# stecrotti/MPSKit.jl

Measured on AMD Instinct MI355X. Metric: DMRG sweeps/sec + ddAC matvec achieved-TFLOP/s, Heisenberg L=100 D=1024 fp64, higher is better.
Workload: dtype f64; 1 GPU; Heisenberg S=1/2 FiniteMPS L=100 D=1024 d=2 W=5 fp64, 1-site DMRG sweep (2L-2 site updates), fixed Krylov budget 8 matvecs/site; parallelism=single GPU

## Files before the change

mpskit.jl_amd/csrc/mpsk_cholqr.hip:

```cpp
#include <hip/hip_runtime.h>
#include <cmath>
#include <cstdio>
#include <cstdlib>
#include <cstring>
#include <string>
#include "mpsk_internal.h"

namespace mpsk {

constexpr int CB = 64;
constexpr double CQ_FIRSTORDER_MAX = 1.0e-7;

__global__ __launch_bounds__(256) void cq_pad_identity_kernel(double* __restrict__ G, int npad, int n) {
  const int64_t total = (int64_t)npad * npad;
  for (int64_t e = blockIdx.x * (int64_t)blockDim.x + threadIdx.x; e < total; e += (int64_t)gridDim.x * blockDim.x) {
    int r = (int)(e % npad), c = (int)(e / npad);
    if (r >= n || c >= n) G[e] = (r == c) ? 1.0 : 0.0;
  }
}

__global__ __launch_bounds__(256) void cq_shift_kernel(double* __restrict__ G, int npad, int n, double factor) {
  __shared__ double red[4];
  __shared__ double sh;
  double acc = 0.0;
// ... 461 lines not shown
    double v = G[r + (int64_t)c * npad] - (r == c ? 1.0 : 0.0);
    if (!(fabs(v) <= thresh)) bad = 1;
  }
  if (bad) atomicOr(flag, 2);
}

static bool cq_use_trsm(int m, int npad) {
  static const bool enabled = !(getenv("MPSK_CQ_TRSM") && atoi(getenv("MPSK_CQ_TRSM")) == 0);
  return enabled && (int64_t)(npad / CB) * ((m + CB - 1) / CB) <= 768;
}
static bool cq_use_gram(int m, int npad) {
  static const bool enabled = !(getenv("MPSK_CQ_GRAM") && atoi(getenv("MPSK_CQ_GRAM")) == 0);
  return enabled && cq_use_trsm(m, npad);
}

size_t cholqr_workspace_doubles(int m, int n) {
  int nb = (n + CB - 1) / CB, p2 = 1;
  while (p2 < nb) p2 <<= 1;
  size_t npad = (size_t)p2 * CB;
  return 5 * npad * npad + 2 * (size_t)m * n + 16 + (cq_use_gram(m, (int)npad) ? (size_t)CQ_GS * npad * npad : 0);
}

static GemmArgs cq_mk(const double* A, const double* B, double* C, int M, int N, int K, int64_t lda, int64_t ldb,
                      int64_t ldc, int tA, double alpha, double beta) {
  GemmArgs g;
  std::memset(&g, 0, sizeof(g));
  g.A = A; g.B = B; g.C = C; g.M = M; g.N = N; g.K = K; g.lda = lda; g.ldb = ldb; g.ldc = ldc;
  g.batch = 1; g.nseg = 1; g.alpha = alpha; g.beta = beta; g.transA = tA; g.transB = 0;
  return g;
}

static hipError_t cq_pass(int m, int n, int npad, const double* X, int ldx, double* Q, int ldq, double* Rp,
                          double* Rinv, double* T, bool shifted, bool check_identity, int* flag, hipStream_t s,
                          double shift_scale = 1.0, bool gram_ready = false, double* Gp_next = nullptr) {
  hipError_t e;
  double* Gw = T;
  GemmArgs g = cq_mk(X, X, Gw, n, n, m, ldx, ldx, npad, 1, 1.0, 0.0);
  g.upper_only = 1;
  if (!gram_ready && (e = gemm_f64(g, s)) != hipSuccess) return e;
  if (npad > n) hipLaunchKernelGGL(cq_pad_identity_kernel, dim3(512), dim3(256), 0, s, Gw, npad, n);
  if (check_identity) hipLaunchKernelGGL(cq_check_identity_kernel, dim3(256), dim3(256), 0, s, Gw, npad, n, 0.5, flag);
  if (shifted) {
    const double u = 1.1102230246251565e-16;
    const double factor = shift_scale * 11.0 * ((double)m * n + (double)n * (n + 1)) * u;
    hipLaunchKernelGGL(cq_shift_kernel, dim3(1), dim3(256), 0, s, Gw, npad, n, factor);
  }
  const int nb = npad / CB;
  static std::atomic<uint64_t> step_attr{0};
  if ((e = ensure_dyn_smem(step_attr, reinterpret_cast<const void*>(cq_step_kernel), CQ_STEP_LDS)) != hipSuccess) return e;
  const bool use_trsm = cq_use_trsm(m, npad);
  if (use_trsm) {
    if (X != Q) {
      if ((e = hipMemcpy2DAsync(Q, sizeof(double) * (size_t)ldq, X, sizeof(double) * (size_t)ldx, sizeof(double) * (size_t)m, n,
                                hipMemcpyDeviceToDevice, s)) != hipSuccess) return e;
    }
    const int mt = (m + CB - 1) / CB;
    for (int k = 0; k <= nb + (Gp_next ? 2 : 1); ++k) {
      const int nt = (nb - k > 0) ? nb - k : 0;
      int nwg = (k == 0) ? 1 : nt * (nt + 1) / 2 + nt;
      if (k - 2 >= 0 && k - 2 < nb) nwg += mt;
      if (k - 3 >= 0 && nb - k + 1 > 0) nwg += (nb - k + 1) * mt;
      if (Gp_next && k - 3 >= 0 && k - 3 < nb) nwg += (k - 2) * CQ_GS;
      if (nwg > 0)
        hipLaunchKernelGGL(cq_step_kernel, dim3(nwg), dim3(256), CQ_STEP_LDS, s, Gw, Rp, Rinv, npad, k, flag, Q, m, n, ldq, 1,
                           Gp_next);
    }
    hipLaunchKernelGGL(cq_cleanup_kernel, dim3(1024), dim3(256), 0, s, Rp, Rinv, npad);
    if (Gp_next) hipLaunchKernelGGL(cq_gram_reduce_kernel, dim3(1024), dim3(256), 0, s, Gp_next, npad, T);
    return hipGetLastError();
  }
  for (int k = 0; k <= nb; ++k) {
    const int nt = nb - k;
    const int pairwg = (k >= 2 && (k & 1) == 0) ? 1 : 0;
    const int nwg = (k == 0) ? 1 : nt * (nt + 1) / 2 + nt + pairwg;
    if (nwg > 0)
      hipLaunchKernelGGL(cq_step_kernel, dim3(nwg), dim3(256), CQ_STEP_LDS, s, Gw, Rp, Rinv, npad, k, flag, (double*)nullptr, 0, 0, 0, 0,
                         (double*)nullptr);
  }
  hipLaunchKernelGGL(cq_cleanup_kernel, dim3(1024), dim3(256), 0, s, Rp, Rinv, npad);
  for (int b = 2 * CB; b < npad; b <<= 1) {
    const int pairs = npad / (2 * b);
    const int64_t bs = (int64_t)2 * b * (npad + 1);
    const int64_t off12 = (int64_t)b * npad;
    const int64_t off22 = (int64_t)b * (npad + 1);
    g = cq_mk(Rp + off12, Rinv + off22, T + off12, b, b, b, npad, npad, npad, 0, 1.0, 0.0);
    g.batch = pairs; g.bsA = bs; g.bsB = bs; g.bsC = bs;
    if ((e = gemm_f64(g, s)) != hipSuccess) return e;
    g = cq_mk(Rinv, T + off12, Rinv + off12, b, b, b, npad, npad, npad, 0, -1.0, 0.0);
    g.batch = pairs; g.bsA = bs; g.bsB = bs; g.bsC = bs;
    if ((e = gemm_f64(g, s)) != hipSuccess) return e;
  }
  g = cq_mk(X, Rinv, Q, m, n, n, ldx, npad, ldq, 0, 1.0, 0.0);
  g.b_upper = 1;
  return gemm_f64(g, s);
}

__global__ __launch_bounds__(256) void cq_copy_upper_kernel(const double* __restrict__ Rp, int npad, int n,
                                                            double* __restrict__ R, int ldr) {
  const int64_t total = (int64_t)n * n;
// ... 16 lines not shown
      if (!(fabs(ev) <= 1.0e-7)) big = 1;
      u = (r < c) ? ev : 0.5 * ev;
    }
    R3[e] = id + u;
    Minv[e] = id - u;
  }
  if (big) atomicOr(flag, 4);
}

static hipError_t cq_pass_firstorder(int m, int n, int npad, const double* X, int ldx, double* Q, int ldq, double* Rp,
                                     double* Rinv, double* T, int* flag, hipStream_t s, bool gram_ready = false) {
  hipError_t e;
  GemmArgs g = cq_mk(X, X, T, n, n, m, ldx, ldx, npad, 1, 1.0, 0.0);
  g.upper_only = 1;
  if (!gram_ready && (e = gemm_f64(g, s)) != hipSuccess) return e;
  hipLaunchKernelGGL(cq_firstorder_kernel, dim3(1024), dim3(256), 0, s, T, npad, n, Rp, Rinv, flag, CQ_FIRSTORDER_MAX);
  g = cq_mk(X, Rinv, Q, m, n, n, ldx, npad, ldq, 0, 1.0, 0.0);
  g.b_upper = 1;
  return gemm_f64(g, s);
}

struct CqBufs { double *R1, *R2, *R3, *Rinv, *T, *Qa, *Qb, *Gp; int npad; };
static CqBufs cq_bufs(int m, int n, double* ws) {
  int nb = (n + CB - 1) / CB, p2 = 1;
  while (p2 < nb) p2 <<= 1;
  CqBufs b;
  b.npad = p2 * CB;
  const size_t np2 = (size_t)b.npad * b.npad;
  b.R1 = ws; b.R2 = b.R1 + np2; b.R3 = b.R2 + np2; b.Rinv = b.R3 + np2; b.T = b.Rinv + np2;
  b.Qa = b.T + np2; b.Qb = b.Qa + (size_t)m * n;
  b.Gp = cq_use_gram(m, b.npad) ? b.Qb + (((size_t)m * n + 1) & ~(size_t)1) : nullptr;
  return b;
}
static hipError_t cq_finish(const CqBufs& b, int n, double* R, int ldr, int* d_flag, int* flag_out, hipStream_t s) {
  hipError_t e;
  GemmArgs g = cq_mk(b.R2, b.R1, b.T, b.npad, b.npad, b.npad, b.npad, b.npad, b.npad, 0, 1.0, 0.0);
  g.a_upper = g.b_upper = g.upper_only = 1;
  if ((e = gemm_f64(g, s)) != hipSuccess) return e;
  g = cq_mk(b.R3, b.T, b.Rinv, b.npad, b.npad, b.npad, b.npad, b.npad, b.npad, 0, 1.0, 0.0);
  g.a_upper = g.b_upper = g.upper_only = 1;
  if ((e = gemm_f64(g, s)) != hipSuccess) return e;
  hipLaunchKernelGGL(cq_copy_upper_kernel, dim3(1024), dim3(256), 0, s, b.Rinv, b.npad, n, R, ldr);
  return hipMemcpyAsync(flag_out, d_flag, sizeof(int), hipMemcpyDeviceToHost, s);
}

static void cq_dbg_count(bool rep) {
  static long n = 0, r = 0;
  if (!getenv("MPSK_CQ_DEBUG")) return;
  ++n; if (rep) ++r;
  if (n % 100 == 0) fprintf(stderr, "[cholqr3] %ld factorizations, %ld repeated the third pass (thr %.1e)\n", n, r, CQ_FIRSTORDER_MAX);
}
hipError_t cholqr3_enqueue(int m, int n, const double* A, int lda, double* Q, int ldq, double* R, int ldr, double* ws,
                           int* d_flag, int* flag_out, hipStream_t s, double shift_scale) {
  const CqBufs b = cq_bufs(m, n, ws);
  hipError_t e;
  if ((e = hipMemsetAsync(d_flag, 0, sizeof(int), s)) != hipSuccess) return e;
  const bool gr = (b.Gp != nullptr);
  if ((e = cq_pass(m, n, b.npad, A, lda, b.Qa, m, b.R1, b.Rinv, b.T, true, false, d_flag, s, shift_scale, false, b.Gp)) != hipSuccess) return e;
  if ((e = cq_pass(m, n, b.npad, b.Qa, m, b.Qb, m, b.R2, b.Rinv, b.T, false, false, d_flag, s, 1.0, gr, b.Gp)) != hipSuccess) return e;
  if ((e = cq_pass_firstorder(m, n, b.npad, b.Qb, m, Q, ldq, b.R3, b.Rinv, b.T, d_flag, s, gr)) != hipSuccess) return e;
  return cq_finish(b, n, R, ldr, d_flag, flag_out, s);
}

hipError_t cholqr3_finalize(int m, int n, double* Q, int ldq, double* R, int ldr, double* ws, int* d_flag,
                            int* flag_out, hipStream_t s) {
  const CqBufs b = cq_bufs(m, n, ws);
  hipError_t e;
  if ((e = hipStreamSynchronize(s)) != hipSuccess) return e;
  cq_dbg_count(*flag_out == 4);
  if (*flag_out == 4) {
    if ((e = hipMemsetAsync(d_flag, 0, sizeof(int), s)) != hipSuccess) return e;
    if ((e = cq_pass(m, n, b.npad, b.Qb, m, Q, ldq, b.R3, b.Rinv, b.T, false, true, d_flag, s)) != hipSuccess) return e;
    if ((e = cq_finish(b, n, R, ldr, d_flag, flag_out, s)) != hipSuccess) return e;
    if ((e = hipStreamSynchronize(s)) != hipSuccess) return e;
  }
  return hipGetLastError();
}

__global__ __launch_bounds__(256) void cq_sumsq_kernel(const double* __restrict__ A, int lda, int m, int n,
                                                       double* __restrict__ out) {
  __shared__ double red[4];
  const int64_t total = (int64_t)m * n;
  double acc = 0.0;
  for (int64_t e = blockIdx.x * (int64_t)blockDim.x + threadIdx.x; e < total; e += (int64_t)gridDim.x * blockDim.x) {
    const double v = A[(e % m) + (e / m) * (int64_t)lda];
    acc += v * v;
  }
  for (int off = 32; off > 0; off >>= 1) acc += __shfl_down(acc, off, 64);
  if ((threadIdx.x & 63) == 0) red[threadIdx.x >> 6] = acc;
  __syncthreads();
  if (threadIdx.x == 0) out[1 + blockIdx.x] = red[0] + red[1] + red[2] + red[3];
}
__global__ __launch_bounds__(64) void cq_sumsq_final_kernel(double* __restrict__ out, int nblocks) {
  if (threadIdx.x == 0) {
    double acc = 0.0;
    for (int i = 0; i < nblocks; ++i) acc += out[1 + i];
    out[0] = acc;
  }
}
__global__ __launch_bounds__(256) void cq_perturb_kernel(const double* __restrict__ A, int lda, int m, int n,
                                                         double* __restrict__ X, int ldx, const double* __restrict__ sumsq) {
  const double delta = 1.1102230246251565e-16 * sqrt(sumsq[0] / (double)m);
  const int64_t total = (int64_t)m * n;
  for (int64_t e = blockIdx.x * (int64_t)blockDim.x + threadIdx.x; e < total; e += (int64_t)gridDim.x * blockDim.x) {
// ... 72 lines not shown
```

mpskit.jl_amd/csrc/mpsk_gemm.hip:

```cpp
#include <hip/hip_runtime.h>
#include <stdint.h>
#include <cstdio>
#include <cstdlib>
#include <cstring>
#include <map>
#include <mutex>
#include <string>
#include <vector>
#include "mpsk_internal.h"

namespace mpsk {

typedef double d4 __attribute__((ext_vector_type(4)));
typedef double d2 __attribute__((ext_vector_type(2)));

constexpr int BK = 16;
constexpr int NTHREADS = 256;

template <int BMN, bool KMAJOR> struct LdsImg {
  static_assert(BK == 16, "the K-major swizzle assumes 128-byte rows");
  static constexpr int STRIDE = KMAJOR ? BK : (BMN + 16);
  static constexpr int SIZE = KMAJOR ? BMN * BK : BK * (BMN + 16);
  __device__ static inline int idx(int mn, int k) { return KMAJOR ? mn * BK + (k ^ (mn & 15)) : k * STRIDE + mn; }
};
// ... 320 lines not shown
    const int rm = tilesM / g.xcd_gx, rn = tilesN / g.xcd_gy;
    const int xi = xcd % g.xcd_gx, yi = xcd / g.xcd_gx;
    const int ln = pos / rm, lm = pos - ln * rm;
    *bm = xi * rm + lm;
    *bn = yi * rn + ln;
    (void)rn;
  } else {
    *bn = t / tilesM;
    *bm = t - *bn * tilesM;
  }
}

template <int BM, int BN, bool ALIGNED, bool CJ = false, bool ZADD = false>
__device__ __forceinline__ void gemm_store_c(const GemmArgs& g, double* __restrict__ Cb, int z, int m0, int n0,
                                             const d4 (&acc)[BM / 32][BN / 32]) {
  constexpr int WTM = BM / 2, WTN = BN / 2, TM = WTM / 16, TN = WTN / 16;
  const int lane = threadIdx.x & 63, wave = threadIdx.x >> 6;
  const int wm = wave & 1, wn = wave >> 1, fr = lane & 15, fq = lane >> 4;
  const double alpha = g.alpha, beta = g.beta;
#pragma unroll
  for (int i = 0; i < TM; ++i) {
    const int m = m0 + wm * WTM + i * 16 + fr;
#pragma unroll
    for (int j = 0; j < TN; ++j) {
#pragma unroll
      for (int rg = 0; rg < 4; ++rg) {
        const int n = n0 + wn * WTN + j * 16 + fq + 4 * rg;
        if (ALIGNED || (m < g.M && n < g.N)) {
          const int64_t mo = CJ ? (int64_t)m * g.c_rs : (int64_t)m;
          double* p = (g.tabC2 != nullptr && n >= g.splitN)
                          ? g.C + g.tabC2[z] + mo + (int64_t)(n - g.splitN) * g.ldc
                          : Cb + mo + (int64_t)n * g.ldc;
          double v = alpha * acc[i][j][rg];
          if constexpr (ZADD) v += g.gamma * g.Z[(int64_t)m + (int64_t)n * g.ldz];
          else if (beta != 0.0) v += beta * (*p);
          *p = v;
        }
      }
    }
  }
}

template <int BM, int BN>
__device__ __forceinline__ void gemm_store_ws(double alpha, double* __restrict__ slot, const d4 (&acc)[BM / 32][BN / 32]) {
  constexpr int WTM = BM / 2, WTN = BN / 2, TM = WTM / 16, TN = WTN / 16;
  const int lane = threadIdx.x & 63, wave = threadIdx.x >> 6;
  const int wm = wave & 1, wn = wave >> 1, fr = lane & 15, fq = lane >> 4;
#pragma unroll
  for (int i = 0; i < TM; ++i)
#pragma unroll
    for (int j = 0; j < TN; ++j)
#pragma unroll
      for (int rg = 0; rg < 4; ++rg)
        slot[(wm * WTM + i * 16 + fr) + (wn * WTN + j * 16 + fq + 4 * rg) * BM] = alpha * acc[i][j][rg];
}

template <int BM, int BN, bool TA, bool TB, bool ALIGNED, bool ZS = false, bool CJ = false, bool ZADD = false>
__device__ __forceinline__ void gemm_body(const GemmArgs& g) {
  extern __shared__ __attribute__((aligned(16))) double smem[];
  const int tilesM = (g.M + BM - 1) / BM, tilesN = (g.N + BN - 1) / BN;
  const int ntiles = tilesM * tilesN;
  int bid = blockIdx.x;
  if (!g.xcd_interleave) {
    int q = ntiles / 8, r = ntiles % 8, xcd = bid % 8, pos = bid / 8;
    bid = (xcd < r ? xcd * (q + 1) : r * (q + 1) + (xcd - r) * q) + pos;
  }
  int bm, bn;
  tile_coords(g, bid, tilesM, tilesN, &bm, &bn);
  const int z = blockIdx.y;
  if (g.upper_only && bm > bn && (g.upper_nb == 0 || z < g.upper_nb)) return;
  const int m0 = bm * BM, n0 = bn * BN;
  const double* Ab = g.A + (g.tabA ? g.tabA[z] : (int64_t)z * g.bsA);
  const double* Bb = g.B + (g.tabB ? g.tabB[z] : (int64_t)z * g.bsB);
  double* Cb = g.C + (g.tabC ? g.tabC[z] : (int64_t)z * g.bsC);
  d4 acc[BM / 32][BN / 32];
#pragma unroll
  for (int i = 0; i < BM / 32; ++i)
#pragma unroll
    for (int j = 0; j < BN / 32; ++j) acc[i][j] = d4{0.0, 0.0, 0.0, 0.0};
  const int nt = ((g.K + BK - 1) / BK) * g.nseg;
  int ktlo = 0, kthi = nt;
  if (g.b_upper) { const int lim = (n0 + BN + BK - 1) / BK; if (lim < kthi) kthi = lim; }
  if (g.a_upper) ktlo = m0 / BK;
  if (ktlo < kthi) gemm_acc_dispatch<BM, BN, TA, TB, ALIGNED, ZS, CJ>(g, Ab, Bb, z, m0, n0, ktlo, kthi, acc, smem);
  gemm_store_c<BM, BN, ALIGNED, CJ, ZADD>(g, Cb, z, m0, n0, acc);
}

template <int BM, int BN, bool TA, bool TB, bool ALIGNED, bool ZS = false, bool ZADD = false>
__device__ __forceinline__ void gemm_sk_body(const GemmArgs& g) {
  extern __shared__ __attribute__((aligned(16))) double smem[];
  constexpr int WTM = BM / 2, WTN = BN / 2, TM = WTM / 16, TN = WTN / 16;
  const int tilesM = (g.M + BM - 1) / BM, tilesN = (g.N + BN - 1) / BN;
  const int ntiles = tilesM * tilesN;
  const int KT = ((g.K + BK - 1) / BK) * g.nseg;
  const int U = ntiles * g.batch * KT;
  int sid = blockIdx.x;
  if (!g.xcd_interleave) {
    const int nwg = gridDim.x;
    int q = nwg / 8, r = nwg % 8, xcd = sid % 8, pos = sid / 8;
    sid = (xcd < r ? xcd * (q + 1) : r * (q + 1) + (xcd - r) * q) + pos;
  }
  int u = sid * g.sk_units;
  int slot = sid;
  if (g.sk_split_major) {
    const int TZ = ntiles * g.batch;
    const int split = sid / TZ, tzs = sid - split * TZ;
    u = tzs * KT + split * g.sk_units;
    slot = tzs * (KT / g.sk_units - 1) + split - 1;
  }
  const int uend = (u + g.sk_units < U) ? u + g.sk_units : U;
  const int lane = threadIdx.x & 63, wave = threadIdx.x >> 6;
  const int wm = wave & 1, wn = wave >> 1, fr = lane & 15, fq = lane >> 4;
  while (u < uend) {
    const int tz = u / KT;
    const int kt0 = u - tz * KT;
    const int kt1 = (uend - u < KT - kt0) ? kt0 + (uend - u) : KT;
    const int z = tz / ntiles, tile = tz - z * ntiles;
    int bm, bn;
// ... 97 lines not shown
      for (int q = 0; q < UNR; ++q) {
        const int e = e0 + 256 * q;
        if (e < eend) sacc[q] += g.sk_ws[(int64_t)(g.sk_split_major ? w - tz - 1 : w) * BM * BN + e];
      }
    }
#pragma unroll
    for (int q = 0; q < UNR; ++q)
      if (pp[q]) *pp[q] = cv[q] + sacc[q];
  }
}

template <int BM, int BN, bool TA, bool TB, bool ALIGNED>
__global__ __launch_bounds__(NTHREADS, min_waves(BM, BN)) void gemm_f64_kernel(GemmArgs g) {
  gemm_body<BM, BN, TA, TB, ALIGNED>(g);
}

template <int BM, int BN, bool ALIGNED>
__global__ __launch_bounds__(NTHREADS, min_waves(BM, BN)) void dac_gemm_f64_kernel(GemmArgs g) {
  gemm_body<BM, BN, false, false, ALIGNED>(g);
}
template <int BM, int BN, bool ALIGNED>
__global__ __launch_bounds__(NTHREADS, min_waves(BM, BN)) void dac_gemm_zs_f64_kernel(GemmArgs g) {
  gemm_body<BM, BN, false, false, ALIGNED, true>(g);
}

template <int BM, int BN, bool ALIGNED>
__global__ __launch_bounds__(NTHREADS, min_waves(BM, BN)) void gemm_tn_zadd_f64_kernel(GemmArgs g) {
  gemm_body<BM, BN, true, false, ALIGNED, false, false, true>(g);
}
template <int BM, int BN, bool ALIGNED>
__global__ __launch_bounds__(NTHREADS, min_waves(BM, BN)) void gemm_tn_zadd_sk_f64_kernel(GemmArgs g) {
  gemm_sk_body<BM, BN, true, false, ALIGNED, false, true>(g);
}

template <int BM, int BN, bool TA, bool TB, bool ALIGNED>
__global__ __launch_bounds__(NTHREADS, min_waves(BM, BN)) void cgemm_f64_kernel(GemmArgs g) {
  gemm_body<BM, BN, TA, TB, ALIGNED, false, true>(g);
}

struct ProfRec { hipEvent_t e0, e1; double flops; int bm, bn, aligned, sk, zs; };
static std::atomic<bool> g_prof_on{false};
static std::atomic<uint64_t> g_prof_seq{0};
static const int g_prof_stride = getenv("MPSK_PROF_STRIDE") && atoi(getenv("MPSK_PROF_STRIDE")) > 0 ? atoi(getenv("MPSK_PROF_STRIDE")) : 1;
static std::mutex g_prof_mu;
static std::vector<ProfRec> g_prof;

void gemm_prof_enable(bool on) {
  std::lock_guard<std::mutex> lk(g_prof_mu);
  if (on && !g_prof_on.load()) {
    for (auto& r : g_prof) { (void)hipEventDestroy(r.e0); (void)hipEventDestroy(r.e1); }
    g_prof.clear();
  }
  if (on) g_prof_seq.store(0);
  g_prof_on.store(on);
}
static void prof_push(const ProfRec& r) {
  std::lock_guard<std::mutex> lk(g_prof_mu);
  g_prof.push_back(r);
}

std::string gemm_prof_summary() {
  (void)hipDeviceSynchronize();
  struct Agg { long n = 0; double ms = 0, flops = 0; };
  std::map<std::string, Agg> agg;
  std::lock_guard<std::mutex> lk(g_prof_mu);
  for (auto& r : g_prof) {
// ... 26 lines not shown
  if (hipError_t e = ensure_dyn_smem(attr, reinterpret_cast<const void*>(kern), smem); e != hipSuccess) return e;
  if (prof) {
    (void)hipEventCreateWithFlags(&r->e0, hipEventDisableSystemFence); (void)hipEventCreateWithFlags(&r->e1, hipEventDisableSystemFence);
    (void)hipEventRecord(r->e0, s);
  }
  hipLaunchKernelGGL(kern, grid, dim3(NTHREADS), smem, s, g);
  return hipGetLastError();
}

template <int BM, int BN, bool TA, bool TB, bool ALIGNED>
static hipError_t launch_cfg(const GemmArgs& g, hipStream_t s) {
  using LA = TileLoader<BM, TA, ALIGNED>;
  using LB = TileLoader<BN, !TB, ALIGNED>;
  constexpr size_t smem = (2 * LA::Img::SIZE + 2 * LB::Img::SIZE) * sizeof(double);
  const int tilesM = (g.M + BM - 1) / BM, tilesN = (g.N + BN - 1) / BN;
  dim3 grid(tilesM * tilesN, g.batch, 1);
  const bool zs = g.zsegA != nullptr;
  if (zs && !(g.tag == 1 && !TA && !TB && g.zsegB != nullptr)) return hipErrorInvalidValue;
  const bool tagged = (g.tag == 1 && !TA && !TB);
  bool prof = tagged && g_prof_on.load(std::memory_order_relaxed);
  if (prof) {
    const uint64_t n = g_prof_seq.fetch_add(1, std::memory_order_relaxed);
    prof = ((n >> 1) % (uint64_t)g_prof_stride) == 0;
  }
  ProfRec r;
  r.flops = 2.0 * g.M * g.N * (double)g.K * g.nseg * g.batch; r.bm = BM; r.bn = BN; r.aligned = ALIGNED; r.sk = 0; r.zs = zs;
  hipError_t e = hipSuccess;
  if (g.cplx) {
    if (zs || g.sk_units > 0) return hipErrorInvalidValue;
    static std::atomic<uint64_t> c0{0};
    return launch_one(cgemm_f64_kernel<BM, BN, TA, TB, ALIGNED>, c0, grid, smem, g, s, false, &r);
  }
  constexpr bool ZADD_OK = TA && !TB;
  if (g.Z && !ZADD_OK) return hipErrorInvalidValue;
  if constexpr ((BM == 128 && BN == 128) || (BM == 64 && BN == 64)) {
    if (g.sk_units > 0) {
      const int KT = ((g.K + BK - 1) / BK) * g.nseg;
      const int64_t U = (int64_t)tilesM * tilesN * g.batch * KT;
      const dim3 sgrid((unsigned)((U + g.sk_units - 1) / g.sk_units));
      r.sk = 1;
      static std::atomic<uint64_t> a0{0}, a1{0}, a2{0}, a3{0};
      if constexpr (ZADD_OK) {
        if (g.Z) e = launch_one(gemm_tn_zadd_sk_f64_kernel<BM, BN, ALIGNED>, a3, sgrid, smem, g, s, false, &r);
        else e = launch_one(gemm_sk_f64_kernel<BM, BN, TA, TB, ALIGNED>, a0, sgrid, smem, g, s, false, &r);
      } else if constexpr (!TA && !TB) {
        if (tagged && zs) e = launch_one(dac_gemm_sk_zs_f64_kernel<BM, BN, ALIGNED>, a2, sgrid, smem, g, s, prof, &r);
        else if (tagged) e = launch_one(dac_gemm_sk_f64_kernel<BM, BN, ALIGNED>, a1, sgrid, smem, g, s, prof, &r);
        else e = launch_one(gemm_sk_f64_kernel<BM, BN, TA, TB, ALIGNED>, a0, sgrid, smem, g, s, false, &r);
      } else {
        e = launch_one(gemm_sk_f64_kernel<BM, BN, TA, TB, ALIGNED>, a0, sgrid, smem, g, s, false, &r);
      }
      if (e != hipSuccess) return e;
      hipLaunchKernelGGL((gemm_sk_fixup_kernel<BM, BN>), dim3(tilesM * tilesN * g.batch, (BM * BN) / 1024), dim3(256), 0, s, g);
      if (prof) { (void)hipEventRecord(r.e1, s); prof_push(r); }
      return hipGetLastError();
    }
  }
  static std::atomic<uint64_t> b0{0}, b1{0}, b2{0}, b3{0};
  if constexpr (ZADD_OK) {
    if (g.Z) e = launch_one(gemm_tn_zadd_f64_kernel<BM, BN, ALIGNED>, b3, grid, smem, g, s, false, &r);
    else e = launch_one(gemm_f64_kernel<BM, BN, TA, TB, ALIGNED>, b0, grid, smem, g, s, false, &r);
  } else if constexpr (!TA && !TB) {
    if (tagged && zs) e = launch_one(dac_gemm_zs_f64_kernel<BM, BN, ALIGNED>, b2, grid, smem, g, s, prof, &r);
    else if (tagged) e = launch_one(dac_gemm_f64_kernel<BM, BN, ALIGNED>, b1, grid, smem, g, s, prof, &r);
    else e = launch_one(gemm_f64_kernel<BM, BN, TA, TB, ALIGNED>, b0, grid, smem, g, s, false, &r);
  } else {
    e = launch_one(gemm_f64_kernel<BM, BN, TA, TB, ALIGNED>, b0, grid, smem, g, s, false, &r);
// ... 37 lines not shown
  std::lock_guard<std::mutex> lk(g_skws_mu);
  SkWs& e = g_skws[std::make_pair(dev, s)];
  if (e.p) return e.p;
  if (hipMalloc(&e.p, SK_WS_DOUBLES * sizeof(double)) != hipSuccess) { e.p = nullptr; return nullptr; }
  return e.p;
}
void gemm_retain_stream(hipStream_t s) {
  int dev = 0;
  if (hipGetDevice(&dev) != hipSuccess) return;
  std::lock_guard<std::mutex> lk(g_skws_mu);
  g_skws[std::make_pair(dev, s)].refs++;
}
void gemm_release_stream(hipStream_t s) {
  int dev = 0;
  if (hipGetDevice(&dev) != hipSuccess) return;
  double* p = nullptr;
  {
    std::lock_guard<std::mutex> lk(g_skws_mu);
    auto it = g_skws.find(std::make_pair(dev, s));
    if (it == g_skws.end()) return;
    if (--it->second.refs > 0) return;
    p = it->second.p;
    g_skws.erase(it);
  }
  if (p) { (void)hipStreamSynchronize(s); (void)hipFree(p); }
}

hipError_t gemm_f64(const GemmArgs& g_in, hipStream_t s) {
  GemmArgs g = g_in;
  if (g.M <= 0 || g.N <= 0 || g.batch <= 0) return hipSuccess;
  if (g.K <= 0 || g.nseg <= 0) {
    return hipErrorInvalidValue;
  }
  if (g.Z && (!g.transA || g.transB || g.cplx || g.tabC2 || g.batch != 1 || g.beta != 0.0 || g.Z == g.C || g.zsegA))
    return hipErrorInvalidValue;
  if (!g.A2 && !g.B2) { g.A2 = g.A; g.B2 = g.B; g.nseg1 = g.nseg; }
  else if (!g.A2 || !g.B2 || !g.zsegA || !g.zsegB || g.nseg1 < 0 || g.nseg1 > g.nseg) return hipErrorInvalidValue;
  int bm = 128, bn = 128;
  choose_tile(g.M, g.N, g.K * g.nseg, g.batch, &bm, &bn);
  g.sk_units = 0;
  g.sk_ws = nullptr;
  g.sk_split_major = 0;
  if (g.cplx && g.c_rs == 0) g.c_rs = 1;
  if (g.upper_only && g.M != g.N) g.upper_only = 0;
  if (g.nseg != 1 || g.transA || g.transB) g.a_upper = g.b_upper = 0;
  if (g_force_bm.load()) { bm = g_force_bm.load(); bn = g_force_bn.load(); }
  else if (g.cplx) {  }
  else {
    const int KT = ((g.K + BK - 1) / BK) * g.nseg;
    const int64_t Tb = (int64_t)((g.M + 127) / 128) * ((g.N + 127) / 128) * g.batch;
    const int64_t Ts = (int64_t)((g.M + 63) / 64) * ((g.N + 63) / 64) * g.batch;
    if (g_sk_enabled) {
      const int64_t Ub = Tb * KT;
      if (Tb >= 128 && Tb < 4 * 512 && Tb % 512 != 0 && Ub / 512 >= 16) {
        double* ws = sk_workspace(s);
        if (ws) { bm = bn = 128; g.sk_units = (int)((Ub + 511) / 512); g.sk_ws = ws; }
      }
    }
    if (g.sk_units == 0 && g_splitk_enabled && bm == 64 && bn == 64 && KT >= 64 && Ts <= 4096) {
      const int64_t slots = (int64_t)(SK_WS_DOUBLES / (64 * 64));
      int best_f = 1;
      double best = 0.0;
      for (int f = 1; f <= 8; ++f) {
        if (f > 1 && (KT / f < 16 || Ts * (f - 1) > slots)) break;
        const int64_t n = (Ts * f + 255) / 256;
        const int r = (int)(n % 4);
        const double phi[4] = {1.0, 0.55, 0.92, 0.98};
        const double len = (double)KT / f + 6.0;
        const double cost = (double)(n - r) * len + (r ? r * len / phi[r] : 0.0) + 3.0 * (f - 1) * (double)n / f + (f > 1 ? 12.0 : 0.0);
        if (f == 1 || cost < 0.97 * best) { best = cost; best_f = f; }
      }
      if (g_splitk_force > 0 && (g_splitk_force == 1 || (KT / g_splitk_force >= 16 && Ts * (g_splitk_force - 1) <= slots)))
        best_f = g_splitk_force;
      if (best_f >= 2) {
        double* ws = sk_workspace(s);
        if (ws) {
          g.sk_units = (KT + best_f - 1) / best_f;
          g.sk_ws = ws;
          g.sk_split_major = (KT % g.sk_units == 0 && KT / g.sk_units == best_f) ? 1 : 0;
          if (!g.sk_split_major) {
// ... 7 lines not shown
  g.xcd_interleave = (g.upper_only || g.a_upper || g.b_upper) ? 1 : 0;
  {
    const int tM = (g.M + bm - 1) / bm, tN = (g.N + bn - 1) / bn;
    g.xcd_gx = g.xcd_gy = 0;
    const bool chunks_ok = ((int64_t)tM * tN) % 8 == 0 &&
                           (g.sk_units == 0 || (((g.K + BK - 1) / BK) * g.nseg) % g.sk_units == 0);
    if (chunks_ok && g_xcd_grid_enabled && !g.xcd_interleave) {
      double best = 0.0;
      const int cand[4][2] = {{1, 8}, {2, 4}, {4, 2}, {8, 1}};
      for (int c = 0; c < 4; ++c) {
        if (tM % cand[c][0] || tN % cand[c][1]) continue;
        const double cost = (double)g.M / cand[c][0] + (double)g.N / cand[c][1];
        if (g.xcd_gx == 0 || cost < best) { best = cost; g.xcd_gx = cand[c][0]; g.xcd_gy = cand[c][1]; }
      }
    }
  }
  bool aligned = (g.M % bm == 0) && (g.N % bn == 0) && (g.K % BK == 0) && (g.lda % 2 == 0) &&
                 (g.ldb % 2 == 0) && (g.bsA % 2 == 0) && (g.bsB % 2 == 0) &&
                 ((uintptr_t)g.A % 16 == 0) && ((uintptr_t)g.B % 16 == 0) &&
                 ((uintptr_t)g.A2 % 16 == 0) && ((uintptr_t)g.B2 % 16 == 0) &&
                 g.lda < ((int64_t)1 << 21) && g.ldb < ((int64_t)1 << 21);
  if (g.tabA || g.tabB || g.zsegA || g.zsegB) aligned = aligned && g.tabs_even;
  if (!g.zsegA) for (int i = 0; i < g.nseg && i < MAXSEG; ++i) aligned = aligned && (g.segA[i] % 2 == 0);
  if (!g.zsegB) for (int i = 0; i < g.nseg && i < MAXSEG; ++i) aligned = aligned && (g.segB[i] % 2 == 0);
  if ((!g.zsegA || !g.zsegB) && g.nseg > MAXSEG) return hipErrorInvalidValue;
  if (g.upper_only && bm != bn) g.upper_only = 0;
#define MPSK_DISPATCH(TA_, TB_)                                                        \
  return aligned ? launch_tile<TA_, TB_, true>(g, bm, bn, s) : launch_tile<TA_, TB_, false>(g, bm, bn, s)
  if (!g.transA && !g.transB) { MPSK_DISPATCH(false, false); }
  if (g.transA && !g.transB) { MPSK_DISPATCH(true, false); }
  if (!g.transA && g.transB) { MPSK_DISPATCH(false, true); }
  MPSK_DISPATCH(true, true);
#undef MPSK_DISPATCH
}

template <int BM, bool ALIGNED, bool TWO> struct PairLoader {
  using L = TileLoader<BM, false, ALIGNED>;
  using Img = typename L::Img;
  static constexpr int NV = L::NV;
  L p, q;
  double c[NV][4];

  __device__ inline void load(const GemmPairArgs& g, int m0, int k0, int tid) {
    p.load(g.P, g.ldp, m0, k0, g.M, g.K, tid);
    if (g.Q) q.load(g.Q, g.ldq, m0, k0, g.M, g.K, tid);
#pragma unroll
    for (int i = 0; i < NV; ++i) {
      const int gk = k0 + (tid + i * NTHREADS) / (BM / 2);
      const bool in = ALIGNED || gk < g.K;
      if (!g.Q) q.r[i] = d2{0.0, 0.0};
      c[i][0] = in ? g.a1[gk] : 0.0;
      c[i][1] = (in && g.Q) ? g.b1[gk] : 0.0;
      c[i][2] = (TWO && in) ? g.a2[gk] : 0.0;
      c[i][3] = (TWO && in && g.Q) ? g.b2[gk] : 0.0;
    }
  }
  __device__ inline void store(double* __restrict__ lds, int tid) const {
#pragma unroll
    for (int i = 0; i < NV; ++i) {
      const int v = tid + i * NTHREADS;
      const int mn = (v % (BM / 2)) * 2, k = v / (BM / 2);
      const d2 pv = p.r[i], qv = q.r[i];
      *reinterpret_cast<d2*>(&lds[Img::idx(mn, k)]) = d2{pv.x * c[i][0] + qv.x * c[i][1], pv.y * c[i][0] + qv.y * c[i][1]};
      if (TWO)
        *reinterpret_cast<d2*>(&lds[Img::SIZE + Img::idx(mn, k)]) =
            d2{pv.x * c[i][2] + qv.x * c[i][3], pv.y * c[i][2] + qv.y * c[i][3]};
// ... 381 lines not shown
```

mpskit.jl_amd/csrc/mpsk_internal.h:

```cpp
#pragma once
#include <hip/hip_runtime.h>
#include <stdint.h>
#include <stddef.h>
#include <atomic>
#include <vector>
#include <string>

namespace mpsk {

inline hipError_t ensure_dyn_smem(std::atomic<uint64_t>& done, const void* kernel, size_t bytes) {
  int dev = 0;
  hipError_t e = hipGetDevice(&dev);
  if (e != hipSuccess) return e;
  const uint64_t bit = 1ull << (dev & 63);
  if (done.load(std::memory_order_acquire) & bit) return hipSuccess;
  e = hipFuncSetAttribute(kernel, hipFuncAttributeMaxDynamicSharedMemorySize, (int)bytes);
  if (e != hipSuccess) return e;
  done.fetch_or(bit, std::memory_order_release);
  return hipSuccess;
}

constexpr int MAXSEG = 32;

struct GemmArgs {
// ... 4 lines not shown
  int64_t lda, ldb, ldc;
  int64_t bsA, bsB, bsC;
  int batch;
  int nseg;
  int64_t segA[MAXSEG], segB[MAXSEG];
  double alpha, beta;
  int transA, transB;
  const int64_t* tabA;
  const int64_t* tabB;
  const int64_t* tabC;
  const int64_t* tabC2;
  int splitN;
  int sk_units;
  int sk_split_major;
  double* sk_ws;
  int xcd_gx, xcd_gy;
  int xcd_interleave;
  const int64_t* zsegA;
  const int64_t* zsegB;
  const double* A2;
  const double* B2;
  int nseg1;
  signed char segJ[MAXSEG];
  int b_upper, a_upper;
  int upper_only;
  int upper_nb;
  int cplx;
  int c_rs;
  int tag;
  int tabs_even;
  const double* Z;
  int64_t ldz;
  double gamma;
};

hipError_t gemm_f64(const GemmArgs& g, hipStream_t s);
void gemm_force_tile(int bm, int bn);
void gemm_retain_stream(hipStream_t s);
void gemm_release_stream(hipStream_t s);
void gemm_enable_streamk(bool on);
void gemm_prof_enable(bool on);
std::string gemm_prof_summary();

struct GemmPairArgs {
  const double* P;
  const double* Q;
  const double* B;
  double* C1;
  double* C2;
  int M, N, K;
  int64_t ldp, ldq, ldb, ld1, ld2;
  const double* a1;
  const double* b1;
  const double* a2;
  const double* b2;
  double beta1, beta2;
};
hipError_t gemm_pair_f64(const GemmPairArgs& g, hipStream_t s);
struct DsumArgs {
  GemmArgs f[2];
  int rmod[2];
  int64_t rstride;
  int ntiles0;
};
static_assert(sizeof(DsumArgs) <= 4096, "DsumArgs is passed by value as a kernel argument");
hipError_t dsum_f64(const DsumArgs& a, hipStream_t s);
hipError_t grassmann_coef(int K, const double* S, double scalar, int mode, double* coef, hipStream_t s);

struct MixTerm { int32_t out, in; double coef; double coef_im = 0.0; };
// ... 96 lines not shown
```

Before: 1.165 sweeps/s.

## Fuse CholeskyQR3 tail: first-order pass, grouped GEMMs, triangular R output

Adds a fused tail path for CholeskyQR3 when the Gram-accumulation buffer exists. The second pass skips its cleanup and Gram-reduce launches, and one kernel reduces the partial Gram, builds the first-order R3 and its inverse, and sets the repeat flag. The Q GEMM and the R2*R1 GEMM then run together in one grouped launch, and the final R3*T product writes straight into R with the lower triangle zeroed (new c_tri epilogue in an NN zadd GEMM path). This removes several kernel launches and a copy kernel per factorization. In exchange it adds new GEMM variants, and the fallback path now needs an extra cleanup launch.

```diff
diff --git a/mpskit.jl_amd/csrc/mpsk_cholqr.hip b/mpskit.jl_amd/csrc/mpsk_cholqr.hip
--- a/mpskit.jl_amd/csrc/mpsk_cholqr.hip
+++ b/mpskit.jl_amd/csrc/mpsk_cholqr.hip
@@ -517,7 +517,8 @@
 
 static hipError_t cq_pass(int m, int n, int npad, const double* X, int ldx, double* Q, int ldq, double* Rp,
                           double* Rinv, double* T, bool shifted, bool check_identity, int* flag, hipStream_t s,
-                          double shift_scale = 1.0, bool gram_ready = false, double* Gp_next = nullptr) {
+                          double shift_scale = 1.0, bool gram_ready = false, double* Gp_next = nullptr,
+                          bool fused_tail = false) {
   hipError_t e;
   double* Gw = T;
   GemmArgs g = cq_mk(X, X, Gw, n, n, m, ldx, ldx, npad, 1, 1.0, 0.0);
@@ -550,6 +551,7 @@
         hipLaunchKernelGGL(cq_step_kernel, dim3(nwg), dim3(256), CQ_STEP_LDS, s, Gw, Rp, Rinv, npad, k, flag, Q, m, n, ldq, 1,
                            Gp_next);
     }
+    if (fused_tail && Gp_next) return hipGetLastError();
     hipLaunchKernelGGL(cq_cleanup_kernel, dim3(1024), dim3(256), 0, s, Rp, Rinv, npad);
     if (Gp_next) hipLaunchKernelGGL(cq_gram_reduce_kernel, dim3(1024), dim3(256), 0, s, Gp_next, npad, T);
     return hipGetLastError();
@@ -632,6 +634,48 @@
   b.Gp = cq_use_gram(m, b.npad) ? b.Qb + (((size_t)m * n + 1) & ~(size_t)1) : nullptr;
   return b;
 }
+static bool cq_use_tail() {
+  static const bool enabled = !(getenv("MPSK_CQ_TAIL") && atoi(getenv("MPSK_CQ_TAIL")) == 0);
+  return enabled;
+}
+__global__ __launch_bounds__(256) void cq_tail_firstorder_kernel(const double* __restrict__ Gp, int npad, int n,
+                                                                 double* __restrict__ R3, double* __restrict__ Minv,
+                                                                 int* __restrict__ flag, double thr) {
+  const int64_t total = (int64_t)npad * npad;
+  int big = 0;
+  for (int64_t e = blockIdx.x * (int64_t)blockDim.x + threadIdx.x; e < total; e += (int64_t)gridDim.x * blockDim.x) {
+    int r = (int)(e % npad), c = (int)(e / npad);
+    double u = 0.0, id = (r == c) ? 1.0 : 0.0;
+    if (r < n && c < n && r <= c) {
+      double acc = 0.0;
+#pragma unroll
+      for (int sp = 0; sp < CQ_GS; ++sp) acc += Gp[(int64_t)sp * total + e];
+      const double ev = acc - id;
+      if (!(fabs(ev) <= thr)) big = 1;
+      u = (r < c) ? ev : 0.5 * ev;
+    }
+    R3[e] = id + u;
+    Minv[e] = id - u;
+  }
+  if (big) atomicOr(flag, 4);
+}
+static hipError_t cq_tail(const CqBufs& b, int m, int n, double* Q, int ldq, double* R, int ldr, int* d_flag, int* flag_out,
+                          hipStream_t s) {
+  hipError_t e;
+  const int npad = b.npad;
+  hipLaunchKernelGGL(cq_tail_firstorder_kernel, dim3(1024), dim3(256), 0, s, b.Gp, npad, n, b.R3, b.Rinv, d_flag, CQ_FIRSTORDER_MAX);
+  GemmArgs gq = cq_mk(b.Qb, b.Rinv, Q, m, n, n, m, npad, ldq, 0, 1.0, 0.0);
+  gq.b_upper = 1;
+  GemmArgs gt = cq_mk(b.R2, b.R1, b.T, npad, npad, npad, npad, npad, npad, 0, 1.0, 0.0);
+  gt.a_upper = gt.b_upper = gt.upper_only = 1;
+  if ((e = gemm_group2_f64(gq, gt, s)) != hipSuccess) return e;
+  GemmArgs gr = cq_mk(b.R3, b.T, R, n, n, n, npad, npad, ldr, 0, 1.0, 0.0);
+  gr.a_upper = gr.b_upper = gr.upper_only = 1;
+  gr.c_tri = 1;
+  if ((e = gemm_f64(gr, s)) != hipSuccess) return e;
+  return hipMemcpyAsync(flag_out, d_flag, sizeof(int), hipMemcpyDeviceToHost, s);
+}
+
 static hipError_t cq_finish(const CqBufs& b, int n, double* R, int ldr, int* d_flag, int* flag_out, hipStream_t s) {
   hipError_t e;
   GemmArgs g = cq_mk(b.R2, b.R1, b.T, b.npad, b.npad, b.npad, b.npad, b.npad, b.npad, 0, 1.0, 0.0);
@@ -656,8 +700,10 @@
   hipError_t e;
   if ((e = hipMemsetAsync(d_flag, 0, sizeof(int), s)) != hipSuccess) return e;
   const bool gr = (b.Gp != nullptr);
+  const bool tail = gr && cq_use_tail();
   if ((e = cq_pass(m, n, b.npad, A, lda, b.Qa, m, b.R1, b.Rinv, b.T, true, false, d_flag, s, shift_scale, false, b.Gp)) != hipSuccess) return e;
-  if ((e = cq_pass(m, n, b.npad, b.Qa, m, b.Qb, m, b.R2, b.Rinv, b.T, false, false, d_flag, s, 1.0, gr, b.Gp)) != hipSuccess) return e;
+  if ((e = cq_pass(m, n, b.npad, b.Qa, m, b.Qb, m, b.R2, b.Rinv, b.T, false, false, d_flag, s, 1.0, gr, b.Gp, tail)) != hipSuccess) return e;
+  if (tail) return cq_tail(b, m, n, Q, ldq, R, ldr, d_flag, flag_out, s);
   if ((e = cq_pass_firstorder(m, n, b.npad, b.Qb, m, Q, ldq, b.R3, b.Rinv, b.T, d_flag, s, gr)) != hipSuccess) return e;
   return cq_finish(b, n, R, ldr, d_flag, flag_out, s);
 }
@@ -670,6 +716,7 @@
   cq_dbg_count(*flag_out == 4);
   if (*flag_out == 4) {
     if ((e = hipMemsetAsync(d_flag, 0, sizeof(int), s)) != hipSuccess) return e;
+    if (b.Gp && cq_use_tail()) hipLaunchKernelGGL(cq_cleanup_kernel, dim3(1024), dim3(256), 0, s, b.R2, b.Rinv, b.npad);
     if ((e = cq_pass(m, n, b.npad, b.Qb, m, Q, ldq, b.R3, b.Rinv, b.T, false, true, d_flag, s)) != hipSuccess) return e;
     if ((e = cq_finish(b, n, R, ldr, d_flag, flag_out, s)) != hipSuccess) return e;
     if ((e = hipStreamSynchronize(s)) != hipSuccess) return e;
diff --git a/mpskit.jl_amd/csrc/mpsk_gemm.hip b/mpskit.jl_amd/csrc/mpsk_gemm.hip
--- a/mpskit.jl_amd/csrc/mpsk_gemm.hip
+++ b/mpskit.jl_amd/csrc/mpsk_gemm.hip
@@ -376,8 +376,10 @@
                           ? g.C + g.tabC2[z] + mo + (int64_t)(n - g.splitN) * g.ldc
                           : Cb + mo + (int64_t)n * g.ldc;
           double v = alpha * acc[i][j][rg];
-          if constexpr (ZADD) v += g.gamma * g.Z[(int64_t)m + (int64_t)n * g.ldz];
-          else if (beta != 0.0) v += beta * (*p);
+          if constexpr (ZADD) {
+            if (g.c_tri && m > n) v = 0.0;
+            else if (g.Z) v += g.gamma * g.Z[(int64_t)m + (int64_t)n * g.ldz];
+          } else if (beta != 0.0) v += beta * (*p);
           *p = v;
         }
       }
@@ -400,11 +402,11 @@
 }
 
 template <int BM, int BN, bool TA, bool TB, bool ALIGNED, bool ZS = false, bool CJ = false, bool ZADD = false>
-__device__ __forceinline__ void gemm_body(const GemmArgs& g) {
+__device__ __forceinline__ void gemm_body_at(const GemmArgs& g, int bid0) {
   extern __shared__ __attribute__((aligned(16))) double smem[];
   const int tilesM = (g.M + BM - 1) / BM, tilesN = (g.N + BN - 1) / BN;
   const int ntiles = tilesM * tilesN;
-  int bid = blockIdx.x;
+  int bid = bid0;
   if (!g.xcd_interleave) {
     int q = ntiles / 8, r = ntiles % 8, xcd = bid % 8, pos = bid / 8;
     bid = (xcd < r ? xcd * (q + 1) : r * (q + 1) + (xcd - r) * q) + pos;
@@ -412,7 +414,11 @@
   int bm, bn;
   tile_coords(g, bid, tilesM, tilesN, &bm, &bn);
   const int z = blockIdx.y;
-  if (g.upper_only && bm > bn && (g.upper_nb == 0 || z < g.upper_nb)) return;
+  bool lower = false;
+  if (g.upper_only && bm > bn && (g.upper_nb == 0 || z < g.upper_nb)) {
+    if constexpr (ZADD) { if (!g.c_tri) return; lower = true; }
+    else return;
+  }
   const int m0 = bm * BM, n0 = bn * BN;
   const double* Ab = g.A + (g.tabA ? g.tabA[z] : (int64_t)z * g.bsA);
   const double* Bb = g.B + (g.tabB ? g.tabB[z] : (int64_t)z * g.bsB);
@@ -426,8 +432,13 @@
   int ktlo = 0, kthi = nt;
   if (g.b_upper) { const int lim = (n0 + BN + BK - 1) / BK; if (lim < kthi) kthi = lim; }
   if (g.a_upper) ktlo = m0 / BK;
+  if (lower) kthi = ktlo;
   if (ktlo < kthi) gemm_acc_dispatch<BM, BN, TA, TB, ALIGNED, ZS, CJ>(g, Ab, Bb, z, m0, n0, ktlo, kthi, acc, smem);
   gemm_store_c<BM, BN, ALIGNED, CJ, ZADD>(g, Cb, z, m0, n0, acc);
+}
+template <int BM, int BN, bool TA, bool TB, bool ALIGNED, bool ZS = false, bool CJ = false, bool ZADD = false>
+__device__ __forceinline__ void gemm_body(const GemmArgs& g) {
+  gemm_body_at<BM, BN, TA, TB, ALIGNED, ZS, CJ, ZADD>(g, blockIdx.x);
 }
 
 template <int BM, int BN, bool TA, bool TB, bool ALIGNED, bool ZS = false, bool ZADD = false>
@@ -591,6 +602,22 @@
 __global__ __launch_bounds__(NTHREADS, min_waves(BM, BN)) void gemm_tn_zadd_sk_f64_kernel(GemmArgs g) {
   gemm_sk_body<BM, BN, true, false, ALIGNED, false, true>(g);
 }
+template <int BM, int BN, bool ALIGNED>
+__global__ __launch_bounds__(NTHREADS, min_waves(BM, BN)) void gemm_nn_zadd_f64_kernel(GemmArgs g) {
+  gemm_body<BM, BN, false, false, ALIGNED, false, false, true>(g);
+}
+
+struct GemmGroup2Args {
+  GemmArgs f[2];
+  int ntiles0;
+};
+static_assert(sizeof(GemmGroup2Args) <= 4096, "GemmGroup2Args is passed by value as a kernel argument");
+template <bool ALIGNED>
+__global__ __launch_bounds__(NTHREADS, min_waves(64, 64)) void gemm_group2_f64_kernel(GemmGroup2Args a) {
+  const int t = blockIdx.x;
+  if (t < a.ntiles0) gemm_body_at<64, 64, false, false, ALIGNED>(a.f[0], t);
+  else gemm_body_at<64, 64, false, false, ALIGNED>(a.f[1], t - a.ntiles0);
+}
 
 template <int BM, int BN, bool TA, bool TB, bool ALIGNED>
 __global__ __launch_bounds__(NTHREADS, min_waves(BM, BN)) void cgemm_f64_kernel(GemmArgs g) {
@@ -683,7 +710,15 @@
     return launch_one(cgemm_f64_kernel<BM, BN, TA, TB, ALIGNED>, c0, grid, smem, g, s, false, &r);
   }
   constexpr bool ZADD_OK = TA && !TB;
-  if (g.Z && !ZADD_OK) return hipErrorInvalidValue;
+  constexpr bool ZADD_NN = !TA && !TB;
+  if (g.Z && !(ZADD_OK || ZADD_NN)) return hipErrorInvalidValue;
+  if constexpr (ZADD_NN) {
+    if (g.Z || g.c_tri) {
+      if (g.sk_units > 0 || zs) return hipErrorInvalidValue;
+      static std::atomic<uint64_t> z0{0};
+      return launch_one(gemm_nn_zadd_f64_kernel<BM, BN, ALIGNED>, z0, grid, smem, g, s, false, &r);
+    }
+  }
   if constexpr ((BM == 128 && BN == 128) || (BM == 64 && BN == 64)) {
     if (g.sk_units > 0) {
       const int KT = ((g.K + BK - 1) / BK) * g.nseg;
@@ -787,7 +822,9 @@
   if (g.K <= 0 || g.nseg <= 0) {
     return hipErrorInvalidValue;
   }
-  if (g.Z && (!g.transA || g.transB || g.cplx || g.tabC2 || g.batch != 1 || g.beta != 0.0 || g.Z == g.C || g.zsegA))
+  if (g.Z && (g.transB || g.cplx || g.tabC2 || g.batch != 1 || g.beta != 0.0 || g.Z == g.C || g.zsegA))
+    return hipErrorInvalidValue;
+  if (g.c_tri && (g.transA || g.transB || g.cplx || g.tabC2 || g.batch != 1 || g.beta != 0.0 || g.zsegA || g.M != g.N))
     return hipErrorInvalidValue;
   if (!g.A2 && !g.B2) { g.A2 = g.A; g.B2 = g.B; g.nseg1 = g.nseg; }
   else if (!g.A2 || !g.B2 || !g.zsegA || !g.zsegB || g.nseg1 < 0 || g.nseg1 > g.nseg) return hipErrorInvalidValue;
@@ -801,6 +838,7 @@
   if (g.nseg != 1 || g.transA || g.transB) g.a_upper = g.b_upper = 0;
   if (g_force_bm.load()) { bm = g_force_bm.load(); bn = g_force_bn.load(); }
   else if (g.cplx) {  }
+  else if ((g.Z && !g.transA) || g.c_tri) {  }
   else {
     const int KT = ((g.K + BK - 1) / BK) * g.nseg;
     const int64_t Tb = (int64_t)((g.M + 127) / 128) * ((g.N + 127) / 128) * g.batch;
@@ -874,6 +912,43 @@
   if (!g.transA && g.transB) { MPSK_DISPATCH(false, true); }
   MPSK_DISPATCH(true, true);
 #undef MPSK_DISPATCH
+}
+
+hipError_t gemm_group2_f64(const GemmArgs& g0, const GemmArgs& g1, hipStream_t s) {
+  GemmGroup2Args a;
+  a.f[0] = g0; a.f[1] = g1;
+  bool aligned = true;
+  int64_t nt[2];
+  for (int f = 0; f < 2; ++f) {
+    GemmArgs& g = a.f[f];
+    if (g.M <= 0 || g.N <= 0 || g.K <= 0 || !g.A || !g.B || !g.C) return hipErrorInvalidValue;
+    if (g.nseg != 1 || g.batch != 1 || g.transA || g.transB || g.cplx || g.Z || g.c_tri || g.tabA || g.tabB || g.tabC ||
+        g.tabC2 || g.zsegA || g.zsegB || g.A2 || g.B2 || g.upper_nb)
+      return hipErrorInvalidValue;
+    g.A2 = g.A; g.B2 = g.B; g.nseg1 = 1;
+    g.sk_units = 0; g.sk_ws = nullptr; g.sk_split_major = 0;
+    g.xcd_gx = g.xcd_gy = 0; g.xcd_interleave = 1;
+    if (g.upper_only && g.M != g.N) g.upper_only = 0;
+    aligned = aligned && (g.M % 64 == 0) && (g.N % 64 == 0) && (g.K % BK == 0) && (g.lda % 2 == 0) && (g.ldb % 2 == 0) &&
+              (g.segA[0] % 2 == 0) && (g.segB[0] % 2 == 0) && ((uintptr_t)g.A % 16 == 0) && ((uintptr_t)g.B % 16 == 0) &&
+              g.lda < ((int64_t)1 << 21) && g.ldb < ((int64_t)1 << 21);
+    nt[f] = (int64_t)((g.M + 63) / 64) * ((g.N + 63) / 64);
+  }
+  if (nt[0] + nt[1] > 0x7fffffff) return hipErrorInvalidValue;
+  a.ntiles0 = (int)nt[0];
+  using IA = LdsImg<64, false>;
+  using IB = LdsImg<64, true>;
+  constexpr size_t smem = (2 * IA::SIZE + 2 * IB::SIZE) * sizeof(double);
+  static std::atomic<uint64_t> done_a{0}, done_u{0};
+  const dim3 grid((unsigned)(nt[0] + nt[1]));
+  if (aligned) {
+    if (hipError_t e = ensure_dyn_smem(done_a, reinterpret_cast<const void*>(gemm_group2_f64_kernel<true>), smem); e != hipSuccess) return e;
+    hipLaunchKernelGGL(gemm_group2_f64_kernel<true>, grid, dim3(NTHREADS), smem, s, a);
+  } else {
+    if (hipError_t e = ensure_dyn_smem(done_u, reinterpret_cast<const void*>(gemm_group2_f64_kernel<false>), smem); e != hipSuccess) return e;
+    hipLaunchKernelGGL(gemm_group2_f64_kernel<false>, grid, dim3(NTHREADS), smem, s, a);
+  }
+  return hipGetLastError();
 }
 
 template <int BM, bool ALIGNED, bool TWO> struct PairLoader {
diff --git a/mpskit.jl_amd/csrc/mpsk_internal.h b/mpskit.jl_amd/csrc/mpsk_internal.h
--- a/mpskit.jl_amd/csrc/mpsk_internal.h
+++ b/mpskit.jl_amd/csrc/mpsk_internal.h
@@ -60,9 +60,11 @@
   const double* Z;
   int64_t ldz;
   double gamma;
+  int c_tri;
 };
 
 hipError_t gemm_f64(const GemmArgs& g, hipStream_t s);
+hipError_t gemm_group2_f64(const GemmArgs& g0, const GemmArgs& g1, hipStream_t s);
 void gemm_force_tile(int bm, int bn);
 void gemm_retain_stream(hipStream_t s);
 void gemm_release_stream(hipStream_t s);
```

Result: no change. 1.175 sweeps/s (median of 6 runs) (+0.9%).
